# jeff-regier/Celeste.jl

Measured on AMD Instinct MI355X. Metric: sources/sec (ELBO value+gradient+Hessian+KL per target source), higher is better.
Workload: dtype f64

## Files before the change

celeste.jl_amd/csrc/celeste_abi.hip:

```cpp
#include <hip/hip_runtime.h>
#include <algorithm>
#include <atomic>
#include <cmath>
#include <cstdio>
#include <cstdlib>
#include <cstring>
#include <mutex>
#include <unordered_map>
#include <vector>

#include "elbo_kernels.h"
#include "optim_kernels.h"
#include "fused_kernels.h"

struct celeste_group;

#define EVAL_FUSED_MAX 32

#define HIP_TRY(expr)                                                                    \
    do {                                                                                 \
        hipError_t e__ = (expr);                                                         \
        if (e__ != hipSuccess) {                                                         \
            fprintf(stderr, "celeste_mi355x: %s failed: %s (%s:%d)\n", #expr,            \
                    hipGetErrorString(e__), __FILE__, __LINE__);                         \
            return CELESTE_ERR_HIP;                                                      \
        }                                                                                \
    } while (0)

static hipError_t celeste_device_malloc(void **p, size_t bytes) {
    hipError_t e = (hipMalloc)(p, bytes);
    static const bool poison = [] { const char *v = getenv("CELESTE_POISON"); return v && atoi(v) != 0; }();
    if (e == hipSuccess && poison) {
        e = hipMemset(*p, 0xFF, bytes);
        if (e == hipSuccess) e = hipDeviceSynchronize();
    }
    return e;
}
#define hipMalloc(p, bytes) celeste_device_malloc((void **)(p), (bytes))

struct StreamPool {
    std::mutex mu;
    std::vector<hipStream_t> idle[16];
};
static StreamPool &stream_pool() { static StreamPool *p = new StreamPool(); return *p; }
static hipError_t stream_acquire(int device, hipStream_t *out) {
    *out = nullptr;
    if (device >= 0 && device < 16) {
        StreamPool &sp = stream_pool();
        std::lock_guard<std::mutex> lk(sp.mu);
        if (!sp.idle[device].empty()) { *out = sp.idle[device].back(); sp.idle[device].pop_back(); return hipSuccess; }
    }
    return hipStreamCreateWithFlags(out, hipStreamNonBlocking);
}
static void stream_retire(int device, hipStream_t s) {
    if (!s) return;
    if (hipStreamSynchronize(s) == hipSuccess && device >= 0 && device < 16) {
        static const size_t cap = [] { const char *e = getenv("CELESTE_STREAM_POOL_MAX"); return e ? (size_t)std::max(0, atoi(e)) : (size_t)32; }();
        StreamPool &sp = stream_pool();
// ... 48 lines not shown
    ;

struct celeste_images {
    int device = 0;
    int N = 0;
    std::vector<DevImage> h_images;
    std::vector<void *> plane_allocs;
    DevImage *d_images = nullptr;
    std::atomic<int> refs{1};
};

static void images_release(celeste_images *im) {
    if (!im || im->refs.fetch_sub(1) != 1) return;
    (void)hipSetDevice(im->device);
    for (void *p : im->plane_allocs) (void)hipFree(p);
    if (im->d_images) (void)hipFree(im->d_images);
    delete im;
}

struct celeste_ctx {
    int device = 0;
    celeste_images *imgs = nullptr;
    hipStream_t stream = nullptr;
    hipStream_t copy_stream = nullptr;
    bool copy_stream_checked = false;
    int N = 0, S = 0, K = 0, NC = 0, n_stamps = 0;
    int chunk_px = 256, CH = 1;
    int max_npx = 0;
    std::vector<DevPatch> h_patches;
    std::vector<int64_t> h_nbr_off;
    std::vector<int32_t> h_nbr_idx;
    DevImage *d_images = nullptr;
    DevPatch *d_patches = nullptr;
    double *d_coefs = nullptr;
    float *d_coefs_f = nullptr;
    uint8_t *d_bitmaps = nullptr;
    int64_t *d_nbr_off = nullptr;
    int32_t *d_nbr_idx = nullptr;
    PriorDev *d_prior = nullptr;
    SrcImg *d_srcimg = nullptr;
    Comp *d_comps = nullptr;
    SrcGeo *d_geo = nullptr;
    int64_t *d_val_off = nullptr;
    double2 *d_val = nullptr;
    int32_t *d_needed = nullptr;
    int32_t stamp = 0;
    std::vector<int32_t> h_vis_off, h_vis_img, h_vis_src;
    int32_t *d_vis_off = nullptr, *d_vis_img = nullptr, *d_vis_src = nullptr;
    int4 *d_value_items = nullptr;
    int4 *d_vitems_src = nullptr;
    int32_t *d_vitem_off = nullptr;
    std::vector<int32_t> h_vitem_off;
    int64_t n_value_items = 0;
    int32_t *d_prep_mark = nullptr;
    double *d_lg_sum = nullptr;
    int64_t *d_nv_base = nullptr;
    int32_t *d_nbr_vis = nullptr;
    int2 *d_items = nullptr;
    size_t items_cap = 0;
    std::vector<int32_t> h_src_chunks;
    std::vector<int64_t> h_top_chunks;
    int max_src_chunks = 0;
    int32_t *d_work = nullptr, *d_work_blk = nullptr, *d_work_total = nullptr;
    size_t work_cap = 0, work_blk_cap = 0;
    int M = 1;
    bool dense = false;
    int64_t V = 0;
    std::vector<int64_t> h_tile_off;
    int64_t *d_tile_off = nullptr;
    int64_t n_tiles = 0;
    int sum_tiles = 4, RCH = 1;
    double *d_rec = nullptr;
    double *d_acc_split = nullptr;
    size_t acc_split_cap = 0;
    double *d_acc = nullptr;
    size_t acc_cap = 0;
    int32_t *d_rec_off = nullptr;
    size_t rec_off_cap = 0;
    double *d_vp = nullptr;
    int32_t *d_targets = nullptr;
    double *d_v = nullptr, *d_d = nullptr, *d_h = nullptr;
    int64_t *d_cnt = nullptr;
    int32_t *d_status = nullptr;
    size_t stage_cap = 0;
    double *p_vp = nullptr;
    int32_t *p_targets = nullptr, *p_status = nullptr;
    double *p_v = nullptr, *p_d = nullptr, *p_h = nullptr;
    int64_t *p_cnt = nullptr;
    size_t pin_cap = 0;
    double *d_small_in = nullptr, *p_small_in = nullptr, *d_small_out = nullptr, *p_small_out = nullptr;
    static const int MAX_PARTS = 8;
    hipEvent_t part_done[MAX_PARTS] = {}, part_copied[MAX_PARTS] = {};
    struct OptBuffers {
        size_t cap = 0;
        double *d_vp = nullptr, *d_v = nullptr, *d_d = nullptr, *d_h = nullptr, *d_H = nullptr, *d_T = nullptr, *d_S = nullptr, *d_pos = nullptr;
        int32_t *d_targets = nullptr, *d_act[2] = {nullptr, nullptr}, *d_evt[2] = {nullptr, nullptr}, *d_count = nullptr,
                *d_st = nullptr;
        void *d_state = nullptr;
        static const int RING = 4;
        double *h_vp = nullptr;
        void *h_state = nullptr;
        int32_t *h_count = nullptr;
        hipEvent_t ev[RING] = {};
    } opt;
    struct FusedBuffers {
        size_t cap_t = 0, cap_rec = 0, cap_q = 0, cap_saved = 0;
// ... 381 lines not shown
        CTX_TRY(dev_upload(&c->d_nv_base, base.data(), base.size()));
        CTX_TRY(dev_upload(&c->d_nbr_vis, nv.data(), nv.size()));
    }
    {
        std::vector<int32_t> sorted(c->h_src_chunks);
        std::sort(sorted.begin(), sorted.end(), [](int32_t a, int32_t b) { return a > b; });
        c->h_top_chunks.assign((size_t)c->S + 1, 0);
        for (int s = 0; s < c->S; ++s) c->h_top_chunks[s + 1] = c->h_top_chunks[s] + sorted[s];
    }
    CTX_TRY(dev_upload<int32_t>(&c->d_work_total, nullptr, 1));
    {
        if (c->N > 0xffff) { celeste_ctx_destroy(c); return CELESTE_ERR_INVALID_ARG; }
        const int n_cls = c->chunk_px / 64;
        std::vector<std::vector<std::pair<int32_t, int32_t>>> by_len(n_cls);
        for (int s = 0; s < c->S; ++s)
            for (int64_t q = c->h_nbr_off[s]; q < c->h_nbr_off[s + 1]; ++q) {
                const int s2 = c->h_nbr_idx[q];
                for (int va = c->h_vis_off[s]; va < c->h_vis_off[s + 1]; ++va) {
                    const int n = c->h_vis_img[va];
                    const int64_t vb = hv(s2, n);
                    if (vb < 0) continue;
                    const DevPatch &a = c->h_patches[va], &b = c->h_patches[vb];
                    const int rh = std::min(a.off_h + a.H2, b.off_h + b.H2) - std::max(a.off_h, b.off_h);
                    const int rw = std::min(a.off_w + a.W2, b.off_w + b.W2 - 1) - std::max(a.off_w, b.off_w);
                    if (rh <= 0 || rw <= 0) continue;
                    const int npx = rh * rw, nch = (npx + c->chunk_px - 1) / c->chunk_px;
                    for (int ch = 0; ch < nch; ++ch) {
                        const int px = std::min(c->chunk_px, npx - ch * c->chunk_px);
                        by_len[n_cls - (px + 63) / 64].push_back({(int32_t)q, (int32_t)(n | (ch << 16))});
                    }
                }
            }
        std::vector<int32_t> link_src(c->h_nbr_idx.size());
        for (int s = 0; s < c->S; ++s)
            for (int64_t q = c->h_nbr_off[s]; q < c->h_nbr_off[s + 1]; ++q) link_src[q] = s;
        std::vector<int4> desc;
        for (auto &v : by_len)
            for (auto &e : v) {
                const int t = link_src[e.first], s2 = c->h_nbr_idx[e.first], n = e.second & 0xffff, ch = e.second >> 16;
                desc.push_back(make_int4((int)hv(s2, n), (int)hv(t, n), ch, t));
            }
        c->n_value_items = (int64_t)desc.size();
        CTX_TRY(dev_upload(&c->d_value_items, desc.data(), desc.size()));
        c->h_vitem_off.assign((size_t)c->S + 1, 0);
        for (auto &d : desc) c->h_vitem_off[(size_t)d.w + 1]++;
        for (int s = 0; s < c->S; ++s) c->h_vitem_off[s + 1] += c->h_vitem_off[s];
        {
            std::vector<int4> by_src(desc.size());
            std::vector<int32_t> fill(c->h_vitem_off.begin(), c->h_vitem_off.end() - 1);
            for (auto &d : desc) by_src[(size_t)fill[d.w]++] = d;
            CTX_TRY(dev_upload(&c->d_vitems_src, by_src.data(), by_src.size()));
            CTX_TRY(dev_upload(&c->d_vitem_off, c->h_vitem_off.data(), c->h_vitem_off.size()));
        }
        CTX_TRY(dev_upload<int32_t>(&c->d_prep_mark, nullptr, (size_t)c->S));
        if (hipMemset(c->d_prep_mark, 0, (size_t)c->S * sizeof(int32_t)) != hipSuccess) { celeste_ctx_destroy(c); return CELESTE_ERR_HIP; }
    }
    {
        c->h_tile_off.resize(c->h_patches.size());
        int64_t tot = 0;
        for (size_t q = 0; q < c->h_patches.size(); ++q) {
            c->h_tile_off[q] = tot;
            tot += ((int64_t)c->h_patches[q].H2 * c->h_patches[q].W2 + 63) / 64;
        }
        c->n_tiles = tot;
        if (const char *e = getenv("CELESTE_SUM_TILES")) if (atoi(e) > 0) c->sum_tiles = atoi(e);
        c->RCH = std::max(1, ((c->max_npx + 63) / 64 + c->sum_tiles - 1) / c->sum_tiles);
    }
    if (hipStreamSynchronize(nullptr) != hipSuccess) { celeste_ctx_destroy(c); return CELESTE_ERR_HIP; }
#undef CTX_TRY
    *out = c;
    return CELESTE_OK;
} ABI_CATCH

extern "C" void celeste_ctx_destroy(celeste_ctx_t *c) {
    if (!c) return;
    (void)hipSetDevice(c->device);
    if (c->stream) (void)hipStreamSynchronize(c->stream);
    if (c->copy_stream) (void)hipStreamSynchronize(c->copy_stream);
    void *ptrs[] = {c->d_patches, c->d_coefs, c->d_coefs_f, c->d_bitmaps, c->d_nbr_off, c->d_nbr_idx, c->d_prior,
                    c->d_srcimg, c->d_comps, c->d_geo, c->d_val_off, c->d_val, c->d_needed, c->d_vis_off, c->d_vis_img, c->d_vis_src, c->d_value_items, c->d_vitems_src, c->d_vitem_off, c->d_prep_mark, c->d_rec_off, c->d_lg_sum, c->d_nv_base, c->d_nbr_vis, c->d_items, c->d_work, c->d_work_blk, c->d_work_total, c->d_tile_off, c->d_rec, c->d_acc_split, c->d_acc, c->d_vp, c->d_targets, c->d_v, c->d_d, c->d_h,
                    c->d_cnt, c->d_status};
    for (void *p : ptrs) if (p) (void)hipFree(p);
    {
        auto &o = c->opt;
        void *optr[] = {o.d_vp, o.d_v, o.d_d, o.d_h, o.d_H, o.d_T, o.d_S, o.d_pos, o.d_targets, o.d_act[0], o.d_act[1], o.d_evt[0], o.d_evt[1],
                        o.d_count, o.d_st, o.d_state};
        for (void *q : optr) if (q) (void)hipFree(q);
        void *hptr[] = {o.h_vp, o.h_state, o.h_count};
        for (void *q : hptr) if (q) staging_free(q);
        for (int k = 0; k < celeste_ctx::OptBuffers::RING; ++k) if (o.ev[k]) (void)hipEventDestroy(o.ev[k]);
        auto &f = c->fused;
        void *fptr[] = {f.d_chunk_desc, f.d_tgt_rec, f.d_q_items, f.d_q_ctl, f.d_arrivals, f.d_saved};
        for (void *q : fptr) if (q) (void)hipFree(q);
        if (f.h_ctl) staging_free(f.h_ctl);
    }
    for (auto &sc : c->scratch) if (sc.p) (void)hipFree(sc.p);
    for (int i = 0; i < 5; ++i) if (c->ev[i]) (void)hipEventDestroy(c->ev[i]);
    for (int i = 0; i < celeste_ctx::MAX_PARTS; ++i) {
        if (c->part_done[i]) (void)hipEventDestroy(c->part_done[i]);
        if (c->part_copied[i]) (void)hipEventDestroy(c->part_copied[i]);
    }
    void *pins[] = {c->p_vp, c->p_targets, c->p_status, c->p_v, c->p_d, c->p_h, c->p_cnt, c->p_small_in, c->p_small_out};
    if (c->d_small_in) (void)hipFree(c->d_small_in);
    if (c->d_small_out) (void)hipFree(c->d_small_out);
    for (void *q : pins) if (q) staging_free(q);
    stream_retire(c->device, c->stream);
    stream_retire(c->device, c->copy_stream);
    images_release(c->imgs);
    delete c;
}

template <class T>
static hipError_t scratch_get(celeste_ctx_t *c, int k, size_t bytes, T **out) {
    auto &s = c->scratch[k];
    if (bytes > s.cap) {
        hipError_t e = s.p ? hipStreamSynchronize(c->stream) : hipSuccess;
        if (e != hipSuccess) return e;
        if (s.p) { (void)hipFree(s.p); s.p = nullptr; s.cap = 0; }
        e = hipMalloc(&s.p, std::max<size_t>(bytes, 256));
        if (e != hipSuccess) return e;
        s.cap = std::max<size_t>(bytes, 256);
    }
    *out = (T *)s.p;
    return hipSuccess;
}

static int launch_eval(celeste_ctx_t *c, const double *d_vp, int32_t n_targets, const int32_t *d_targets,
                       uint32_t flags, double *d_v, double *d_d, double *d_h, int64_t *d_counters, int32_t *d_status,
                       void *stream_, bool render_neighbors, const int32_t *d_active_rank = nullptr,
                       int64_t n_chunks = -1, bool tables_current = false, const int32_t *d_live = nullptr,
                       bool prep_all = false, bool render_only = false, const int32_t *d_h_pos = nullptr);

extern "C" int celeste_elbo_eval_batch_device(celeste_ctx_t *c, const double *d_vp, int32_t n_targets,
// ... 130 lines not shown
    const size_t setup_threads = std::max<size_t>(render_neighbors ? (size_t)c->S : 0, (size_t)n_targets * (c->dense ? 1 : c->M));
    int32_t *const prep_mark = render_neighbors && !tables_current && !prep_all ? c->d_prep_mark : nullptr;
    bool prep_fused = false;
    bool records_described = false;
    if (eval_fused) { int stb = fused_buffers(c, (size_t)n_targets, rec_cap, stream); if (stb != CELESTE_OK) return stb; }
    if (n_visits <= WORK1_MAX_VISITS && !getenv("CELESTE_PARALLEL_WORKLIST")) {
        const unsigned setup_blocks = (unsigned)((setup_threads + WORK1_SETUP - 1) / WORK1_SETUP);
        prep_fused = !render_neighbors && !getenv("CELESTE_NO_FUSED_PREP");
        const bool prep_all_here = render_neighbors && !tables_current && c->V > 0 && c->V <= WORK1_PREP_ALL_MAX &&
                                   (n_targets >= WORK1_PREP_ALL_MIN_TARGETS || c->V <= WORK1_PREP_ALL_TINY) && !getenv("CELESTE_NO_FUSED_PREP");
        const int prep_n = prep_all_here ? (int)c->V : n_visits;
        if (prep_all_here) prep_fused = true;
        const unsigned prep_blocks = prep_fused ? (unsigned)((prep_n + WORK1_NT / 64 - 1) / (WORK1_NT / 64)) : 0u;
        const bool records_described_here = eval_fused && c->dense && !d_live && !getenv("CELESTE_NO_FUSED_DESCRIBE");
        hipLaunchKernelGGL(setup_worklist_kernel, dim3(1 + setup_blocks + prep_blocks), dim3(WORK1_NT),
                           0, stream, d_vp, geo_S, c->d_geo, d_targets, n_targets, c->d_vis_off, c->d_vis_img, c->M,
                           c->dense ? nullptr : c->d_items, render_neighbors ? c->d_needed : nullptr, c->stamp, c->d_patches,
                           c->N, CH, chunk_px, G, (int)c->dense, c->d_work, c->d_work_total, d_live, prep_mark,
                           c->d_nbr_off, c->d_nbr_idx, c->d_rec_off, (int)setup_blocks, c->d_images, c->K, c->d_srcimg,
                           c->d_comps, prep_all_here ? (int)c->V : 0, c->d_vis_src,
                           records_described_here ? c->fused.d_chunk_desc : nullptr, records_described_here ? c->fused.d_tgt_rec : nullptr,
                           c->chunk_px);
        records_described = records_described_here;
    } else {
        hipLaunchKernelGGL(setup_kernel, dim3((unsigned)((setup_threads + 63) / 64)), dim3(64), 0, stream, d_vp, geo_S,
                           c->d_geo, d_targets, n_targets, c->d_vis_off, c->d_vis_img, c->M, c->dense ? nullptr : c->d_items,
                           render_neighbors ? c->d_needed : nullptr, c->stamp, prep_mark, c->d_nbr_off, c->d_nbr_idx, d_live);
        hipLaunchKernelGGL(work_count_kernel, dim3(n_wblk), dim3(WORK_NT), 0, stream, d_targets, n_visits, c->d_patches,
                           c->d_vis_off, c->d_vis_img, c->N, c->M, chunk_px, G, (int)c->dense, c->d_work_blk, d_live);
        hipLaunchKernelGGL(work_scan_kernel, dim3(1), dim3(1024), 0, stream, c->d_work_blk, n_wblk * (n_classes + 1),
                           c->d_work_total, n_wblk * n_classes);
        hipLaunchKernelGGL(work_fill_kernel, dim3(n_wblk), dim3(WORK_NT), 0, stream, d_targets, n_visits, c->d_patches,
                           c->d_vis_off, c->d_vis_img, c->N, c->M, CH, chunk_px, G, (int)c->dense, c->d_work_blk, c->d_work, d_live,
                           c->d_rec_off);
    }
    if (render_neighbors) {
        if (c->V > 0 && !tables_current && !prep_fused)
            hipLaunchKernelGGL(prep_kernel, dim3((unsigned)c->V), dim3(64), 0, stream, d_vp, c->d_images, c->d_patches,
                               c->d_vis_src, c->d_vis_img, c->N, c->K, c->d_srcimg, c->d_comps, nullptr, c->d_vis_off, c->M,
                               (int)c->dense, nullptr, prep_mark, c->stamp);
    } else if (!prep_fused) {
        hipLaunchKernelGGL(prep_kernel, dim3((unsigned)std::max(n_visits, 1)), dim3(64), 0, stream, d_vp, c->d_images,
                           c->d_patches, c->d_vis_src, c->d_vis_img, c->N, c->K, c->d_srcimg, c->d_comps, d_targets,
                           c->d_vis_off, c->M, (int)c->dense, d_live, nullptr, 0);
    }
    if (render_neighbors) {
    if (c->n_value_items > 0)
    {
        const bool wide_items = n_targets <= VALUE_WIDE_MAX && c->chunk_px == 256 && !getenv("CELESTE_NO_WIDE_VALUE");
#define LAUNCH_VALUE(R, WAVES)                                                                                              \
        hipLaunchKernelGGL((value_kernel<R, WAVES>), dim3((unsigned)c->n_value_items), dim3(64 * WAVES), 0, stream,       \
                           c->d_patches, c->d_coefs, c->d_srcimg, c->d_comps, c->d_needed, c->stamp, c->d_val_off,          \
                           c->d_value_items, c->NC, c->chunk_px, c->d_val, c->d_coefs_f)
        if (flags & CELESTE_FLAG_FP32) { if (wide_items) LAUNCH_VALUE(float, 2); else LAUNCH_VALUE(float, 1); }
        else { if (wide_items) LAUNCH_VALUE(double, 4); else LAUNCH_VALUE(double, 1); }
#undef LAUNCH_VALUE
    }
    }
    if (render_only) { HIP_TRY(hipGetLastError()); return CELESTE_OK; }
    if (c->timing) HIP_TRY(hipEventRecord(c->ev[1], stream));
    if (eval_fused) {
        auto &fb = c->fused;
        if (fb.arrivals_dirty) {
            HIP_TRY(hipMemsetAsync(fb.d_arrivals, 0, fb.cap_t * sizeof(int32_t), stream));
            fb.arrivals_dirty = false;
        }
        if (!records_described)
            hipLaunchKernelGGL(fused_setup_kernel, dim3((unsigned)((n_targets + 63) / 64)), dim3(64), 0, stream, d_targets, n_targets,
                               c->d_patches, c->d_vis_off, c->dense ? nullptr : c->d_items, c->N, c->M, c->chunk_px, c->d_rec_off,
                               fb.d_chunk_desc, fb.d_tgt_rec, (int32_t *)nullptr, (int32_t *)nullptr);
        FusedArgs A;
        fused_args_tables(c, A);
        A.targets = d_targets; A.n_targets = n_targets; A.vp = const_cast<double *>(d_vp);
        A.chunk_desc = fb.d_chunk_desc; A.tgt_rec = fb.d_tgt_rec; A.arrivals = fb.d_arrivals; A.flags = flags;
        memset(&A.op, 0, sizeof A.op);
        const unsigned rec_bound = (unsigned)std::max<size_t>(n_chunks >= 0 ? grid_need : work_need, 1);
        hipLaunchKernelGGL(eval_fused_kernel, dim3(rec_bound + (unsigned)n_targets), dim3(FUSED_NT), 0, stream, A, c->d_srcimg,
                           c->d_comps, c->d_work_total, (int)rec_bound, d_v, d_d, d_h, d_counters, d_status);
        if (c->timing) { HIP_TRY(hipEventRecord(c->ev[2], stream)); HIP_TRY(hipEventRecord(c->ev[3], stream)); c->ev_valid = 1; c->ev_split = 0; }
        HIP_TRY(hipGetLastError());
        return CELESTE_OK;
    }
    const dim3 grid((unsigned)std::max<size_t>(grid_need, 1));
#define PIXEL_ARGS                                                                                                \
    c->d_images, c->d_patches, c->d_coefs, c->d_bitmaps, c->d_srcimg, c->d_comps, c->d_nbr_off, c->d_nbr_idx,       \
    c->d_val_off, c->d_val, d_targets, c->N, c->NC, CH, chunk_px, G, c->d_acc, c->d_tile_off, c->d_rec, \
    d_active_rank, c->d_items, c->M, c->d_work, c->d_work_total, c->d_nv_base, c->d_nbr_vis, c->d_rec_off, c->d_coefs_f
#define LAUNCH_PIXEL_T(MODE, R) hipLaunchKernelGGL((pixel_kernel<MODE, R>), grid, dim3(64), 0, stream, PIXEL_ARGS)
#define LAUNCH_PIXEL_M(MODE) hipLaunchKernelGGL((pixel_kernel<MODE, double, true>), grid, dim3(64), 0, stream, PIXEL_ARGS)
#define LAUNCH_PIXEL(MODE) do { if (flags & CELESTE_FLAG_FP32) LAUNCH_PIXEL_T(MODE, float); else LAUNCH_PIXEL_T(MODE, double); } while (0)
    if (d_active_rank) {
        if (flags & CELESTE_FLAG_HESS) LAUNCH_PIXEL_M(2);
        else if (derivs) LAUNCH_PIXEL_M(1);
        else LAUNCH_PIXEL_M(0);
    }
    else if (split) LAUNCH_PIXEL(3);
    else if (flags & CELESTE_FLAG_HESS) LAUNCH_PIXEL(2);
    else if (derivs) LAUNCH_PIXEL(1);
    else LAUNCH_PIXEL_T(0, double);
#undef LAUNCH_PIXEL
#undef LAUNCH_PIXEL_M
#undef PIXEL_ARGS
#undef LAUNCH_PIXEL_T
    if (c->timing) HIP_TRY(hipEventRecord(c->ev[2], stream));
    c->ev_split = 0;
    const int lift_nt = n_targets <= 1024 ? 512 : 256;
    bool lift7 = n_targets > 4096;
    if (const char *e = getenv("CELESTE_LIFT_WAVES")) lift7 = atoi(e) == 7;
// ... 1065 lines not shown
```

celeste.jl_amd/csrc/elbo_kernels.h:

```cpp
#pragma once
#include <hip/hip_runtime.h>
#include <math.h>
#include "elbo_device.h"
#include "../../include/celeste_mi355x.h"

#ifndef CELESTE_MUTANT
#define CELESTE_MUTANT 0
#endif

__constant__ double c_eta[16];
__constant__ double c_nu[16];

__device__ inline void bvn_cov(double ab, double angle, double scale, double &x11, double &x12, double &x22) {
    double sp, cp;
    sincos(angle, &sp, &cp);
    double ab_term = ab * ab - 1.0;
    double s2 = scale * scale;
    x12 = -s2 * cp * sp * ab_term;
    x11 = s2 * (1.0 + ab_term * (sp * sp));
    x22 = s2 * (1.0 + ab_term * (cp * cp));
}

__device__ inline void brightness(const double *vs, int i, int b, double &El, double &Ell) {
    const double r = vs[6 + i], v = vs[8 + i];
// ... 691 lines not shown
    const int k0 = threadIdx.x * per, k1 = min(n_visits, k0 + per);
    const int lane = threadIdx.x & 63, wv = threadIdx.x >> 6;
    constexpr int NCL = WORK_CLASSES + 1;
    int cnt[NCL];
#pragma unroll
    for (int c = 0; c < NCL; ++c) cnt[c] = 0;
    for (int k = k0; k < k1; ++k) {
        int n_full, lc, nch;
        visit_chunks(k, targets, patches, vis_off, vis_img, N, M, chunk_px, G, dense != 0, n_full, lc, &nch);
        cnt[0] += n_full;
#pragma unroll
        for (int c = 1; c < WORK_CLASSES; ++c) cnt[c] += lc == c;
        cnt[WORK_CLASSES] += nch;
    }
    int off[NCL];
    if (threadIdx.x == 0) s_base[0] = 0;
#pragma unroll
    for (int c = 0; c < NCL; ++c) {
        int x = cnt[c];
#pragma unroll
        for (int d = 1; d < 64; d <<= 1) { const int y = __shfl_up(x, d); if (lane >= d) x += y; }
        __syncthreads();
        if (lane == 63) s_part[wv] = x;
        __syncthreads();
        int before = 0, tot = 0;
#pragma unroll
        for (int w = 0; w < WORK1_NT / 64; ++w) { const int v = s_part[w]; before += w < wv ? v : 0; tot += v; }
        off[c] = before + x - cnt[c];
        if (threadIdx.x == 0) s_base[c + 1] = s_base[c] + tot;
    }
    __syncthreads();
    if (threadIdx.x == 0) *work_total = s_base[WORK_CLASSES];
#pragma unroll
    for (int c = 0; c < WORK_CLASSES; ++c) off[c] += s_base[c];
    for (int k = k0; k < k1; ++k) {
        int n_full, lc, nch;
        visit_chunks(k, targets, patches, vis_off, vis_img, N, M, chunk_px, G, dense != 0, n_full, lc, &nch);
        for (int g = 0; g < n_full; ++g) work[off[0]++] = k * CH + g * G;
#pragma unroll
        for (int c = 1; c < WORK_CLASSES; ++c) if (lc == c) work[off[c]++] = k * CH + n_full * G;
        rec_off[k] = off[WORK_CLASSES];
        off[WORK_CLASSES] += nch;
    }
    if (fz_tgt_rec) {
        __syncthreads();
        for (int ti = threadIdx.x; ti < n_targets; ti += WORK1_NT) {
            int first;
            const int n_rec = describe_target_records(ti, targets[ti], patches, nullptr, N, M, fz_chunk_px, rec_off, fz_chunk_desc, first);
            fz_tgt_rec[ti] = make_int2(first < 0 ? 0 : first, n_rec);
        }
    }
}

template <bool COH, typename R = double>
__device__ __forceinline__ void value_pixels(int lane, const DevPatch &P, const SrcImg &si, const Comp *__restrict__ tc, int NC,
                                             const double *__restrict__ coefs, const double *__restrict__ etab, int h_lo,
                                             int w_lo, int RH, int p0, int p1, double2 *__restrict__ out,
                                             const float *__restrict__ tcf = nullptr) {
    const double *__restrict__ coef = coefs + (size_t)(CELESTE_MUTANT == 3 ? 0 : P.stamp) * (CEL_COEF * CEL_COEF);
    const double sh0 = 26.0 - si.m1, sw0 = 26.0 - si.m2;
    const float rRH = 1.0f / (float)RH;
    for (int idx = p0 + lane; idx < p1; idx += 64) {
        int rw, rh;
        divmod_small(idx, RH, rRH, rw, rh);
        const int h0 = h_lo + rh, w0 = w_lo + rw;
        const double hh = (double)(h0 + 1), ww = (double)(w0 + 1);
        double f0, f1;
        if constexpr (sizeof(R) == 8) {
            f0 = star_value(coef, hh + sh0, ww + sw0);
            f1 = galaxy_value(tc, NC, hh - si.m1, ww - si.m2, etab);
        } else {
            f0 = (double)star_value_f(coef, (float)(hh + sh0), (float)(ww + sw0));
            f1 = (double)galaxy_value_f(tcf, NC, (float)(hh - si.m1), (float)(ww - si.m2));
        }
        const double En = si.c0 * f0 + si.c1 * f1;
        const double E2n = si.q0 * (f0 * f0) + si.q1 * (f1 * f1);
        double2 *const o = out + ((h0 - P.off_h) + (int64_t)P.H2 * (w0 - P.off_w));
        const double var = E2n - En * En;
        if constexpr (COH) { stc<true>(&o->x, En); stc<true>(&o->y, var); }
        else *o = make_double2(En, var);
    }
}

typedef float f2v __attribute__((ext_vector_type(2)));
__device__ __forceinline__ void value_pixels_f2(int lane, const DevPatch &P, const SrcImg &si, int NC, const float *__restrict__ coef,
                                                int h_lo, int w_lo, int RH, int p0, int p1, double2 *__restrict__ out,
                                                const float *__restrict__ tcf) {
    const double sh0 = 26.0 - si.m1, sw0 = 26.0 - si.m2;
    const float rRH = 1.0f / (float)RH;
    const f2v *tp = reinterpret_cast<const f2v *>(tcf);
    const int n_dev = 8 * (NC / 14);
    for (int base = p0; base < p1; base += 128) {
        int h0[2], w0[2];
        bool ok[2];
        float dxs[2], dys[2], xh[2], xw[2];
#pragma unroll
        for (int q = 0; q < 2; ++q) {
            const int i = base + 64 * q + lane;
            ok[q] = i < p1;
            int rw, rh;
            divmod_small(min(i, p1 - 1), RH, rRH, rw, rh);
            h0[q] = h_lo + rh; w0[q] = w_lo + rw;
            const double hh = (double)(h0[q] + 1), ww = (double)(w0[q] + 1);
            dxs[q] = (float)(hh - si.m1); dys[q] = (float)(ww - si.m2);
            xh[q] = (float)(hh + sh0); xw[q] = (float)(ww + sw0);
        }
        const f2v dx = {dxs[0], dxs[1]}, dy = {dys[0], dys[1]};
        f2v f1 = (f2v)(0.0f);
        for (int c0 = 0; c0 < NC; c0 += (c0 < n_dev ? 8 : 6)) {
            const int len = c0 < n_dev ? 8 : 6;
            const f2v *k0 = tp + 3 * c0;
            const f2v d1 = dx - k0[3].xx, d2 = dy - k0[4].xx;
            const f2v s11 = -0.72134752044448170368f * (d1 * d1), s12 = -1.44269504088896340736f * (d1 * d2),
                      s22 = -0.72134752044448170368f * (d2 * d2);
            for (int c = c0; c < c0 + len; c += 2) {
                const f2v *k = tp + 3 * c;
                {
                    const f2v p11 = k[0].xx, p12 = k[1].xx, p22 = k[2].xx, w = k[5].xx;
                    const f2v q2 = p11 * s11 + (p12 * s12 + p22 * s22);
                    f1 += w * (f2v){__builtin_amdgcn_exp2f(q2.x), __builtin_amdgcn_exp2f(q2.y)};
                }
                {
                    const f2v p11 = k[0].yy, p12 = k[1].yy, p22 = k[2].yy, w = k[5].yy;
                    const f2v q2 = p11 * s11 + (p12 * s12 + p22 * s22);
                    f1 += w * (f2v){__builtin_amdgcn_exp2f(q2.x), __builtin_amdgcn_exp2f(q2.y)};
                }
            }
        }
        const float *cc[2];
        float fxs[2], fys[2];
#pragma unroll
        for (int q = 0; q < 2; ++q) {
            int ix = (int)floorf(xh[q]); ix = ix < 1 ? 1 : (ix > 50 ? 50 : ix);
            int iy = (int)floorf(xw[q]); iy = iy < 1 ? 1 : (iy > 50 ? 50 : iy);
            cc[q] = coef + (ix - 1) + CEL_COEF * (iy - 1);
            fxs[q] = xh[q] - (float)ix; fys[q] = xw[q] - (float)iy;
        }
        f2v wx[4], wy[4];
        bspline_w((f2v){fxs[0], fxs[1]}, wx); bspline_w((f2v){fys[0], fys[1]}, wy);
        f2v y = (f2v)(0.0f);
#pragma unroll
        for (int b = 0; b < 4; ++b) {
            const float *ca = cc[0] + CEL_COEF * b, *cb = cc[1] + CEL_COEF * b;
            const f2v r = (f2v){ca[0], cb[0]} * wx[0] + (f2v){ca[1], cb[1]} * wx[1] + (f2v){ca[2], cb[2]} * wx[2] + (f2v){ca[3], cb[3]} * wx[3];
            y += r * wy[b];
        }
        const float f0s[2] = {y.x < 0 ? 1e-3f * __expf(y.x) : 1e-3f * (y.x + 1.0f), y.y < 0 ? 1e-3f * __expf(y.y) : 1e-3f * (y.y + 1.0f)};
        const float f1s[2] = {f1.x, f1.y};
#pragma unroll
        for (int q = 0; q < 2; ++q) {
            if (!ok[q]) continue;
            const double f0 = (double)f0s[q], g1 = (double)f1s[q];
            const double En = si.c0 * f0 + si.c1 * g1;
            const double E2n = si.q0 * (f0 * f0) + si.q1 * (g1 * g1);
            out[(h0[q] - P.off_h) + (int64_t)P.H2 * (w0[q] - P.off_w)] = make_double2(En, E2n - En * En);
        }
    }
}

#ifdef VALUE_TIMING
__device__ unsigned long long g_value_clk[8];
#endif
template <typename R, int WAVES = 1>
__global__ void __launch_bounds__(64 * WAVES)
value_kernel(const DevPatch *__restrict__ patches, const double *__restrict__ coefs,
             const SrcImg *__restrict__ srcimg, const Comp *__restrict__ comps,
             const int32_t *__restrict__ is_target, int32_t stamp, const int64_t *__restrict__ val_off,
             const int4 *__restrict__ items, int NC, int chunk_px, double2 *__restrict__ val,
             const float *__restrict__ coefs_f) {
    __shared__ double etab[64];
#ifdef VALUE_TIMING
    long long vts[4]; vts[0] = clock64();
#define VT(k) do { vts[(k) + 1] = clock64(); } while (0)
#else
#define VT(k) do { } while (0)
#endif
    const int4 it = items[blockIdx.x];
    const int sn = it.x, ch = it.z, t = it.w;
    if (is_target[t] != stamp) return;
    const DevPatch &P = patches[sn];
    const DevPatch &T = patches[it.y];
    const int h_lo = max(P.off_h, T.off_h), h_hi = min(P.off_h + P.H2, T.off_h + T.H2);
    const int w_lo = max(P.off_w, T.off_w), w_hi = min(P.off_w + P.W2 - 1, T.off_w + T.W2);
    const int RH = h_hi - h_lo, RW = w_hi - w_lo;
    if (RH <= 0 || RW <= 0) return;
    const int npx = RH * RW;
    const int p0 = ch * chunk_px;
    if (p0 >= npx) return;
    VT(0);
    exp_table_init(etab);
    const int p1 = min(npx, p0 + chunk_px);
    const SrcImg si = srcimg[sn];
    __shared__ Comp tc[14 * CEL_MAXK];
    {
        const double *src = reinterpret_cast<const double *>(comps + (size_t)sn * NC);
        double *dst = reinterpret_cast<double *>(tc);
        for (int i = threadIdx.x; i < NC * 8; i += 64 * WAVES) dst[i] = src[i];
        __syncthreads();
    }
    __shared__ float tcf[sizeof(R) == 4 ? 6 * 14 * CEL_MAXK : 2];
    if constexpr (sizeof(R) == 4) {
        if ((int)threadIdx.x < NC) {
            const Comp k = tc[threadIdx.x];
            float *o = tcf + 12 * (threadIdx.x >> 1) + (threadIdx.x & 1);
            o[0] = (float)k.p11; o[2] = (float)k.p12; o[4] = (float)k.p22; o[6] = (float)k.xi1; o[8] = (float)k.xi2; o[10] = (float)k.w0;
        }
        __syncthreads();
    }
    VT(1);
    if constexpr (sizeof(R) == 4) {
        const int q0 = p0 + 128 * (int)(threadIdx.x >> 6);
        if (WAVES == 1 || q0 < p1)
            value_pixels_f2(threadIdx.x & 63, P, si, NC, coefs_f + (size_t)(CELESTE_MUTANT == 3 ? 0 : P.stamp) * (CEL_COEF * CEL_COEF), h_lo, w_lo, RH,
                            WAVES == 1 ? p0 : q0, WAVES == 1 ? p1 : min(p1, q0 + 128), val + val_off[sn], tcf);
    } else if constexpr (WAVES == 1)
        value_pixels<false, R>(threadIdx.x, P, si, tc, NC, coefs, etab, h_lo, w_lo, RH, p0, p1, val + val_off[sn], tcf);
    else {
        const int q0 = p0 + 64 * (int)(threadIdx.x >> 6);
        if (q0 < p1) value_pixels<false, R>(threadIdx.x & 63, P, si, tc, NC, coefs, etab, h_lo, w_lo, RH, q0, min(p1, q0 + 64), val + val_off[sn], tcf);
    }
    VT(2);
#ifdef VALUE_TIMING
    if (threadIdx.x == 0) {
        for (int k = 0; k < 3; ++k) atomicAdd(&g_value_clk[k], (unsigned long long)(vts[k + 1] - vts[k]));
        atomicAdd(&g_value_clk[7], 1ull); atomicAdd(&g_value_clk[6], (unsigned long long)((p1 - p0 + 63) / 64));
    }
#endif
#undef VT
}

template <typename S>
struct PixelTermsT {
    typedef S scalar;
    S vterm, cnt_act, cnt_inact;
    S f0, f1;
    S alpha, beta, w2, w12;
    S k0, k1;
    S f0g0, f0g1, f0h0, f0h1, f0h2;
    S C0s, C0g, C1s, C1g;
    S Q0s, Q0g, Q1s, Q1g;
    S Wgg, Wsg, Wss;
    S S0d, S1x, S1y, S1xd, S1yd, S2a, S2b, S2c, S2an, S2bn, S2cn, S2ad, S2bd, S2cd;
    S S3a, S3b, S3c, S3d, S4a, S4b, S4c, S4d, S4e;
};
typedef PixelTermsT<double> PixelTerms;

template <int G, class TT>
__device__ __forceinline__ typename TT::scalar gal_g(const TT &T) {
    typedef typename TT::scalar S;
    if constexpr (G == 0) return T.S1x;
    else if constexpr (G == 1) return T.S1y;
    else if constexpr (G == 2) return T.S0d;
    else if constexpr (G == 3) return (S)0.5 * T.S2an;
    else if constexpr (G == 4) return T.S2bn;
    else return (S)0.5 * T.S2cn;
}
template <int G, int G2, class TT>
__device__ __forceinline__ typename TT::scalar gal_h(const TT &T) {
    typedef typename TT::scalar S;
    constexpr int k = G * 6 + G2;
    if constexpr (k == 0) return T.S2a;
    else if constexpr (k == 1) return T.S2b;
    else if constexpr (k == 2) return T.S1xd;
    else if constexpr (k == 3) return (S)0.5 * T.S3a;
    else if constexpr (k == 4) return T.S3b;
    else if constexpr (k == 5) return (S)0.5 * T.S3c;
    else if constexpr (k == 7) return T.S2c;
    else if constexpr (k == 8) return T.S1yd;
    else if constexpr (k == 9) return (S)0.5 * T.S3b;
    else if constexpr (k == 10) return T.S3c;
    else if constexpr (k == 11) return (S)0.5 * T.S3d;
    else if constexpr (k == 14) return (S)0.0;
    else if constexpr (k == 15) return (S)0.5 * T.S2ad;
    else if constexpr (k == 16) return T.S2bd;
    else if constexpr (k == 17) return (S)0.5 * T.S2cd;
    else if constexpr (k == 21) return (S)0.25 * T.S4a;
    else if constexpr (k == 22) return (S)0.5 * T.S4b;
    else if constexpr (k == 23) return (S)0.25 * T.S4c;
    else if constexpr (k == 28) return T.S4c;
    else if constexpr (k == 29) return (S)0.5 * T.S4d;
    else { static_assert(k == 35, "upper triangle only"); return (S)0.25 * T.S4e; }
// ... 1795 lines not shown
```

Before: 3.027 million.

## Render neighbor values per source as deduplicated pixel union tiles

Adds a tile-based value kernel that, for each neighbor source patch, precomputes the union of pixels overlapping any linked target patch and renders each such pixel once, instead of once per (neighbor, target) link item. This removes redundant evaluation of overlapping pixels across links. It adds packed pixel lists, link tables and a per-pixel check against active targets when only some linked targets are active. It is used when wide items are not selected.

```diff
diff --git a/celeste.jl_amd/csrc/celeste_abi.hip b/celeste.jl_amd/csrc/celeste_abi.hip
--- a/celeste.jl_amd/csrc/celeste_abi.hip
+++ b/celeste.jl_amd/csrc/celeste_abi.hip
@@ -4,6 +4,7 @@
 #include <cmath>
 #include <cstdio>
 #include <cstdlib>
+#include <climits>
 #include <cstring>
 #include <mutex>
 #include <unordered_map>
@@ -158,6 +159,12 @@
     int32_t *d_vitem_off = nullptr;
     std::vector<int32_t> h_vitem_off;
     int64_t n_value_items = 0;
+    int4 *d_tile_items = nullptr;
+    uint32_t *d_tile_pix = nullptr;
+    int64_t *d_tile_pix_off = nullptr;
+    int32_t *d_tile_link_off = nullptr;
+    int2 *d_tile_links = nullptr;
+    int64_t n_tile_items = 0;
     int32_t *d_prep_mark = nullptr;
     double *d_lg_sum = nullptr;
     int64_t *d_nv_base = nullptr;
@@ -645,6 +652,54 @@
             CTX_TRY(dev_upload(&c->d_vitems_src, by_src.data(), by_src.size()));
             CTX_TRY(dev_upload(&c->d_vitem_off, c->h_vitem_off.data(), c->h_vitem_off.size()));
         }
+        {
+            std::vector<std::vector<int2>> tl(c->h_patches.size());
+            for (auto &d : desc) if (d.z == 0) tl[(size_t)d.x].push_back(make_int2(d.w, d.y));
+            std::vector<int64_t> pix_off(1, 0);
+            std::vector<int32_t> link_off(1, 0);
+            std::vector<uint32_t> pix;
+            std::vector<int2> links;
+            const int n_cls = c->chunk_px / 64;
+            std::vector<std::vector<int4>> by_len(n_cls);
+            std::vector<int> lo, hi;
+            bool packable = true;
+            for (size_t vb = 0; vb < tl.size(); ++vb) {
+                if (tl[vb].empty()) continue;
+                const DevPatch &b = c->h_patches[vb];
+                if (b.off_h < 0 || b.off_w < 0 || b.off_h + b.H2 > 0xffff || b.off_w + b.W2 > 0xffff) { packable = false; break; }
+                lo.assign((size_t)b.W2, INT_MAX); hi.assign((size_t)b.W2, INT_MIN);
+                for (const int2 &l : tl[vb]) {
+                    const DevPatch &a = c->h_patches[(size_t)l.y];
+                    const int h0 = std::max(a.off_h, b.off_h), h1 = std::min(a.off_h + a.H2, b.off_h + b.H2);
+                    const int w0 = std::max(a.off_w, b.off_w), w1 = std::min(a.off_w + a.W2, b.off_w + b.W2 - 1);
+                    for (int w = w0; w < w1; ++w) {
+                        lo[(size_t)(w - b.off_w)] = std::min(lo[(size_t)(w - b.off_w)], h0);
+                        hi[(size_t)(w - b.off_w)] = std::max(hi[(size_t)(w - b.off_w)], h1);
+                    }
+                }
+                const int u = (int)pix_off.size() - 1;
+                const size_t first = pix.size();
+                for (int w = 0; w < b.W2; ++w)
+                    for (int h = lo[(size_t)w]; h < hi[(size_t)w]; ++h) pix.push_back((uint32_t)h | ((uint32_t)(b.off_w + w) << 16));
+                const int npx = (int)(pix.size() - first);
+                pix_off.push_back((int64_t)pix.size());
+                links.insert(links.end(), tl[vb].begin(), tl[vb].end());
+                link_off.push_back((int32_t)links.size());
+                for (int p0 = 0; p0 < npx; p0 += c->chunk_px) {
+                    const int px = std::min(c->chunk_px, npx - p0);
+                    by_len[(size_t)(n_cls - (px + 63) / 64)].push_back(make_int4((int)vb, u, p0, 0));
+                }
+            }
+            if (!packable) for (auto &v : by_len) v.clear();
+            std::vector<int4> items;
+            for (auto &v : by_len) items.insert(items.end(), v.begin(), v.end());
+            c->n_tile_items = (int64_t)items.size();
+            CTX_TRY(dev_upload(&c->d_tile_items, items.data(), items.size()));
+            CTX_TRY(dev_upload(&c->d_tile_pix, pix.data(), c->n_tile_items ? pix.size() : 0));
+            CTX_TRY(dev_upload(&c->d_tile_pix_off, pix_off.data(), pix_off.size()));
+            CTX_TRY(dev_upload(&c->d_tile_links, links.data(), links.size()));
+            CTX_TRY(dev_upload(&c->d_tile_link_off, link_off.data(), link_off.size()));
+        }
         CTX_TRY(dev_upload<int32_t>(&c->d_prep_mark, nullptr, (size_t)c->S));
         if (hipMemset(c->d_prep_mark, 0, (size_t)c->S * sizeof(int32_t)) != hipSuccess) { celeste_ctx_destroy(c); return CELESTE_ERR_HIP; }
     }
@@ -671,7 +726,7 @@
     if (c->stream) (void)hipStreamSynchronize(c->stream);
     if (c->copy_stream) (void)hipStreamSynchronize(c->copy_stream);
     void *ptrs[] = {c->d_patches, c->d_coefs, c->d_coefs_f, c->d_bitmaps, c->d_nbr_off, c->d_nbr_idx, c->d_prior,
-                    c->d_srcimg, c->d_comps, c->d_geo, c->d_val_off, c->d_val, c->d_needed, c->d_vis_off, c->d_vis_img, c->d_vis_src, c->d_value_items, c->d_vitems_src, c->d_vitem_off, c->d_prep_mark, c->d_rec_off, c->d_lg_sum, c->d_nv_base, c->d_nbr_vis, c->d_items, c->d_work, c->d_work_blk, c->d_work_total, c->d_tile_off, c->d_rec, c->d_acc_split, c->d_acc, c->d_vp, c->d_targets, c->d_v, c->d_d, c->d_h,
+                    c->d_srcimg, c->d_comps, c->d_geo, c->d_val_off, c->d_val, c->d_needed, c->d_vis_off, c->d_vis_img, c->d_vis_src, c->d_value_items, c->d_tile_items, c->d_tile_pix, c->d_tile_pix_off, c->d_tile_link_off, c->d_tile_links, c->d_vitems_src, c->d_vitem_off, c->d_prep_mark, c->d_rec_off, c->d_lg_sum, c->d_nv_base, c->d_nbr_vis, c->d_items, c->d_work, c->d_work_blk, c->d_work_total, c->d_tile_off, c->d_rec, c->d_acc_split, c->d_acc, c->d_vp, c->d_targets, c->d_v, c->d_d, c->d_h,
                     c->d_cnt, c->d_status};
     for (void *p : ptrs) if (p) (void)hipFree(p);
     {
@@ -908,8 +963,17 @@
         hipLaunchKernelGGL((value_kernel<R, WAVES>), dim3((unsigned)c->n_value_items), dim3(64 * WAVES), 0, stream,       \
                            c->d_patches, c->d_coefs, c->d_srcimg, c->d_comps, c->d_needed, c->stamp, c->d_val_off,          \
                            c->d_value_items, c->NC, c->chunk_px, c->d_val, c->d_coefs_f)
-        if (flags & CELESTE_FLAG_FP32) { if (wide_items) LAUNCH_VALUE(float, 2); else LAUNCH_VALUE(float, 1); }
-        else { if (wide_items) LAUNCH_VALUE(double, 4); else LAUNCH_VALUE(double, 1); }
+#define LAUNCH_TILE(R)                                                                                                      \
+        hipLaunchKernelGGL((tile_value_kernel<R>), dim3((unsigned)c->n_tile_items), dim3(64), 0, stream, c->d_patches,    \
+                           c->d_coefs, c->d_srcimg, c->d_comps, c->d_needed, c->stamp, c->d_val_off, c->d_tile_items,       \
+                           c->d_tile_pix_off, c->d_tile_pix, c->d_tile_link_off, c->d_tile_links, c->NC, c->chunk_px,       \
+                           c->d_val, c->d_coefs_f)
+        if (flags & CELESTE_FLAG_FP32) {
+            if (wide_items) LAUNCH_VALUE(float, 2); else if (c->n_tile_items > 0) LAUNCH_TILE(float); else LAUNCH_VALUE(float, 1);
+        } else {
+            if (wide_items) LAUNCH_VALUE(double, 4); else if (c->n_tile_items > 0) LAUNCH_TILE(double); else LAUNCH_VALUE(double, 1);
+        }
+#undef LAUNCH_TILE
 #undef LAUNCH_VALUE
     }
     }
diff --git a/celeste.jl_amd/csrc/elbo_kernels.h b/celeste.jl_amd/csrc/elbo_kernels.h
--- a/celeste.jl_amd/csrc/elbo_kernels.h
+++ b/celeste.jl_amd/csrc/elbo_kernels.h
@@ -767,18 +767,26 @@
     }
 }
 
-template <bool COH, typename R = double>
-__device__ __forceinline__ void value_pixels(int lane, const DevPatch &P, const SrcImg &si, const Comp *__restrict__ tc, int NC,
-                                             const double *__restrict__ coefs, const double *__restrict__ etab, int h_lo,
-                                             int w_lo, int RH, int p0, int p1, double2 *__restrict__ out,
-                                             const float *__restrict__ tcf = nullptr) {
+struct RectLocator {
+    int h_lo, w_lo, RH;
+    float rRH;
+    __device__ RectLocator(int h_lo_, int w_lo_, int RH_) : h_lo(h_lo_), w_lo(w_lo_), RH(RH_), rRH(1.0f / (float)RH_) {}
+    __device__ __forceinline__ bool operator()(int idx, int &h0, int &w0) const {
+        int rw, rh;
+        divmod_small(idx, RH, rRH, rw, rh);
+        h0 = h_lo + rh; w0 = w_lo + rw;
+        return true;
+    }
+};
+template <bool COH, typename R, typename Loc>
+__device__ __forceinline__ void value_pixels_at(int lane, const DevPatch &P, const SrcImg &si, const Comp *__restrict__ tc, int NC,
+                                                const double *__restrict__ coefs, const double *__restrict__ etab, const Loc &loc,
+                                                int p0, int p1, double2 *__restrict__ out, const float *__restrict__ tcf) {
     const double *__restrict__ coef = coefs + (size_t)(CELESTE_MUTANT == 3 ? 0 : P.stamp) * (CEL_COEF * CEL_COEF);
     const double sh0 = 26.0 - si.m1, sw0 = 26.0 - si.m2;
-    const float rRH = 1.0f / (float)RH;
     for (int idx = p0 + lane; idx < p1; idx += 64) {
-        int rw, rh;
-        divmod_small(idx, RH, rRH, rw, rh);
-        const int h0 = h_lo + rh, w0 = w_lo + rw;
+        int h0, w0;
+        if (!loc(idx, h0, w0)) continue;
         const double hh = (double)(h0 + 1), ww = (double)(w0 + 1);
         double f0, f1;
         if constexpr (sizeof(R) == 8) {
@@ -796,13 +804,20 @@
         else *o = make_double2(En, var);
     }
 }
+template <bool COH, typename R = double>
+__device__ __forceinline__ void value_pixels(int lane, const DevPatch &P, const SrcImg &si, const Comp *__restrict__ tc, int NC,
+                                             const double *__restrict__ coefs, const double *__restrict__ etab, int h_lo,
+                                             int w_lo, int RH, int p0, int p1, double2 *__restrict__ out,
+                                             const float *__restrict__ tcf = nullptr) {
+    value_pixels_at<COH, R>(lane, P, si, tc, NC, coefs, etab, RectLocator(h_lo, w_lo, RH), p0, p1, out, tcf);
+}
 
 typedef float f2v __attribute__((ext_vector_type(2)));
-__device__ __forceinline__ void value_pixels_f2(int lane, const DevPatch &P, const SrcImg &si, int NC, const float *__restrict__ coef,
-                                                int h_lo, int w_lo, int RH, int p0, int p1, double2 *__restrict__ out,
-                                                const float *__restrict__ tcf) {
+template <typename Loc>
+__device__ __forceinline__ void value_pixels_f2_at(int lane, const DevPatch &P, const SrcImg &si, int NC, const float *__restrict__ coef,
+                                                   const Loc &loc, int p0, int p1, double2 *__restrict__ out,
+                                                   const float *__restrict__ tcf) {
     const double sh0 = 26.0 - si.m1, sw0 = 26.0 - si.m2;
-    const float rRH = 1.0f / (float)RH;
     const f2v *tp = reinterpret_cast<const f2v *>(tcf);
     const int n_dev = 8 * (NC / 14);
     for (int base = p0; base < p1; base += 128) {
@@ -812,10 +827,8 @@
 #pragma unroll
         for (int q = 0; q < 2; ++q) {
             const int i = base + 64 * q + lane;
-            ok[q] = i < p1;
-            int rw, rh;
-            divmod_small(min(i, p1 - 1), RH, rRH, rw, rh);
-            h0[q] = h_lo + rh; w0[q] = w_lo + rw;
+            const bool need = loc(min(i, p1 - 1), h0[q], w0[q]);
+            ok[q] = i < p1 && need;
             const double hh = (double)(h0[q] + 1), ww = (double)(w0[q] + 1);
             dxs[q] = (float)(hh - si.m1); dys[q] = (float)(ww - si.m2);
             xh[q] = (float)(hh + sh0); xw[q] = (float)(ww + sw0);
@@ -871,6 +884,11 @@
             out[(h0[q] - P.off_h) + (int64_t)P.H2 * (w0[q] - P.off_w)] = make_double2(En, E2n - En * En);
         }
     }
+}
+__device__ __forceinline__ void value_pixels_f2(int lane, const DevPatch &P, const SrcImg &si, int NC, const float *__restrict__ coef,
+                                                int h_lo, int w_lo, int RH, int p0, int p1, double2 *__restrict__ out,
+                                                const float *__restrict__ tcf) {
+    value_pixels_f2_at(lane, P, si, NC, coef, RectLocator(h_lo, w_lo, RH), p0, p1, out, tcf);
 }
 
 #ifdef VALUE_TIMING
@@ -942,6 +960,68 @@
     }
 #endif
 #undef VT
+}
+
+struct TileLocator {
+    const uint32_t *__restrict__ pix;
+    bool all;
+    const DevPatch *__restrict__ patches; const DevPatch *P; const int2 *__restrict__ links; int l0, l1;
+    const int32_t *__restrict__ is_target; int32_t stamp;
+    __device__ __forceinline__ bool operator()(int idx, int &h0, int &w0) const {
+        const uint32_t c = pix[idx];
+        h0 = (int)(c & 0xffffu); w0 = (int)(c >> 16);
+        if (all) return true;
+        bool need = false;
+        for (int l = l0; l < l1; ++l) {
+            const int2 lk = links[l];
+            if (is_target[lk.x] != stamp) continue;
+            const DevPatch &T = patches[lk.y];
+            need |= h0 >= max(P->off_h, T.off_h) && h0 < min(P->off_h + P->H2, T.off_h + T.H2) &&
+                    w0 >= max(P->off_w, T.off_w) && w0 < min(P->off_w + P->W2 - 1, T.off_w + T.W2);
+        }
+        return need;
+    }
+};
+template <typename R>
+__global__ void __launch_bounds__(64)
+tile_value_kernel(const DevPatch *__restrict__ patches, const double *__restrict__ coefs,
+                  const SrcImg *__restrict__ srcimg, const Comp *__restrict__ comps,
+                  const int32_t *__restrict__ is_target, int32_t stamp, const int64_t *__restrict__ val_off,
+                  const int4 *__restrict__ items, const int64_t *__restrict__ pix_off, const uint32_t *__restrict__ pix,
+                  const int32_t *__restrict__ link_off, const int2 *__restrict__ links, int NC, int chunk_px,
+                  double2 *__restrict__ val, const float *__restrict__ coefs_f) {
+    __shared__ double etab[64];
+    const int4 it = items[blockIdx.x];
+    const int sn = it.x, u = it.y, p0 = it.z;
+    const int l0 = link_off[u], l1 = link_off[u + 1];
+    int n_act = 0;
+    for (int l = l0; l < l1; ++l) n_act += is_target[links[l].x] == stamp;
+    if (n_act == 0) return;
+    const int64_t q0 = pix_off[u];
+    const int p1 = (int)min(pix_off[u + 1] - q0, (int64_t)(p0 + chunk_px));
+    const DevPatch &P = patches[sn];
+    const TileLocator loc{pix + q0, n_act == l1 - l0, patches, &P, links, l0, l1, is_target, stamp};
+    exp_table_init(etab);
+    const SrcImg si = srcimg[sn];
+    __shared__ Comp tc[14 * CEL_MAXK];
+    {
+        const double *src = reinterpret_cast<const double *>(comps + (size_t)sn * NC);
+        double *dst = reinterpret_cast<double *>(tc);
+        for (int i = threadIdx.x; i < NC * 8; i += 64) dst[i] = src[i];
+        __syncthreads();
+    }
+    __shared__ float tcf[sizeof(R) == 4 ? 6 * 14 * CEL_MAXK : 2];
+    if constexpr (sizeof(R) == 4) {
+        if ((int)threadIdx.x < NC) {
+            const Comp k = tc[threadIdx.x];
+            float *o = tcf + 12 * (threadIdx.x >> 1) + (threadIdx.x & 1);
+            o[0] = (float)k.p11; o[2] = (float)k.p12; o[4] = (float)k.p22; o[6] = (float)k.xi1; o[8] = (float)k.xi2; o[10] = (float)k.w0;
+        }
+        __syncthreads();
+        value_pixels_f2_at(threadIdx.x, P, si, NC, coefs_f + (size_t)(CELESTE_MUTANT == 3 ? 0 : P.stamp) * (CEL_COEF * CEL_COEF), loc,
+                           p0, p1, val + val_off[sn], tcf);
+    } else
+        value_pixels_at<false, R>(threadIdx.x, P, si, tc, NC, coefs, etab, loc, p0, p1, val + val_off[sn], tcf);
 }
 
 template <typename S>
```

Measured after the change: 3.075 million, median of 6. 1.6% higher.
